# jeongminpark417/COALA-GNN

Measured on AMD Instinct MI355X. Metric: feature-gather GB/s (payload = rows x dim x 4 B delivered per second), IGB-medium GraphSAGE minibatch fetch, higher is better.
Workload: dtype f32

## Files before the change

coala-gnn_amd/csrc/coala_cache.hip:

```cpp
#include <hip/hip_runtime.h>
#include <hip/hip_ext.h>

#include <algorithm>
#include <cstdarg>
#include <cstdio>
#include <cstdlib>
#include <cstring>
#include <new>
#include <type_traits>
#include <utility>
#include <vector>

#include "../../include/coala_hip.h"
#include "coala_internal.h"

namespace {

constexpr uint64_t kEmptyKey = 0xFFFFFFFFFFFFFFFFull;
constexpr uint32_t kLinkMiss = 0x80000000u;
constexpr uint32_t kLinkBad = 0x7FFFFFFFu;
constexpr int kStatBlocks = 2048;
constexpr int kFillSlots = 8;

struct CacheDev {
    void* keys;
    uint64_t* set_cnt;
    uint32_t* color_meta;
    int32_t* color_counters;
    const int32_t* node_color;
    float* lines;
    const float* cold;
    uint64_t num_sets;
    uint64_t num_rows;
    uint32_t cache_dim;
    uint32_t dim;
    uint32_t n_gpus;
    int32_t gshift;
    int32_t sshift;
    uint32_t distributed;
    uint32_t cold_partitioned;
    uint32_t tag32;
    uint64_t* set_head;
    uint32_t* miss_link;
    unsigned long long* stats;
};

__device__ __forceinline__ uint64_t set_of(const CacheDev& c, uint64_t id) {
    uint64_t k = id;
    if (c.distributed) {
        if (c.gshift >= 0) k = id >> c.gshift;
        else if ((id >> 32) == 0) k = (uint32_t)id / c.n_gpus;
        else k = id / c.n_gpus;
    }
    if (c.sshift >= 0) return k & (c.num_sets - 1);
    if ((k >> 32) == 0 && (c.num_sets >> 32) == 0) return (uint32_t)k % (uint32_t)c.num_sets;
    return k % c.num_sets;
}

__device__ __forceinline__ uint64_t cold_row_of(const CacheDev& c, uint64_t id) {
    if (!c.cold_partitioned) return id;
    if (c.gshift >= 0) return id >> c.gshift;
    return id / c.n_gpus;
}

constexpr int kMaxRanges = 64;
struct RangeSet {
    uint32_t n;
    uint32_t total;
    uint32_t begin[kMaxRanges];
    uint32_t vstart[kMaxRanges + 1];
};
__device__ __forceinline__ uint32_t pos_of(const RangeSet& rs, uint32_t v) {
    if (rs.n == 1) return v < rs.total ? rs.begin[0] + v : 0xFFFFFFFFu;
    uint32_t pos = 0xFFFFFFFFu;
    for (uint32_t k = 0; k < rs.n; ++k) {
        const uint32_t a = rs.vstart[k], b = rs.vstart[k + 1];
        if (v >= a && v < b) pos = rs.begin[k] + (v - a);
    }
// ... 48 lines not shown
    static constexpr int UNITS = CD / VEC;
    static constexpr int LPR = UNITS >= 64 ? 64 : UNITS;
    static constexpr int RPP = 64 / LPR;
    static constexpr int VPL = UNITS / LPR;
    static constexpr int PASSES = (VPL >= 16) ? 1 : NP;
    static constexpr int R = RPP * PASSES;
};

constexpr int kK1MinWaves = 4;
constexpr int kK1Passes = 4;
constexpr int64_t kK1SingleMaxChunks = 1 << 20;
constexpr int kK1Waves = 2;
#ifdef COALA_DEV_KNOBS
constexpr int kK1MaxWaves = 4;
#else
constexpr int kK1MaxWaves = kK1Waves;
#endif

template <typename V> __device__ __forceinline__ V nt_load(const V* p) { return __builtin_nontemporal_load(p); }
template <typename V> __device__ __forceinline__ void nt_store(V v, V* p) { __builtin_nontemporal_store(v, p); }

template <int CD, int VEC, typename TAG, int NP, bool FULL, bool REDIR, bool SINGLE>
__global__ __launch_bounds__(64 * kK1MaxWaves, kK1MinWaves) void probe_gather_kernel(const int64_t* __restrict__ idx, float* __restrict__ out,
                                                                    int64_t n, uint32_t gen, uint32_t n_blocks, CacheDev c, Redirect rd) {
    using G = Geo<CD, VEC, NP>;
    using V = typename VecT<VEC>::type;
    using TG = TagGeo<TAG>;
    using TV = typename TG::vec;
    constexpr int R = G::R;
    static_assert(R <= 32, "per-chunk row masks are 32 bits wide");
    if (blockIdx.x == 0 && threadIdx.x < kFillSlots) reinterpret_cast<uint32_t*>(c.stats + 2 * kStatBlocks)[(gen & 1u) * kFillSlots + threadIdx.x] = 0u;
    uint32_t* fill_flag = reinterpret_cast<uint32_t*>(c.stats + 2 * kStatBlocks) + 2 * kFillSlots;
    if (blockIdx.x == 0 && threadIdx.x == kFillSlots) fill_flag[(gen + 1u) & 1u] = 0u;
    constexpr int TSTEPS = (R + TG::SPL - 1) / TG::SPL;
    int lane = threadIdx.x & 63;
#ifdef COALA_DEV_KNOBS
    const int wpb = (int)(blockDim.x >> 6);
#else
    constexpr int wpb = kK1Waves;
#endif
    const int64_t wave = (int64_t)blockIdx.x * wpb + (threadIdx.x >> 6);
    const int64_t n_waves = (int64_t)n_blocks * wpb;
    const int64_t n_chunks = (n + R - 1) / R;
    const uint32_t nunits = c.dim / VEC;
    const TAG* __restrict__ keys = reinterpret_cast<const TAG*>(c.keys);

    struct Ids { uint64_t id[TSTEPS]; bool valid[TSTEPS]; int32_t drow[REDIR ? TSTEPS : 1]; };
    struct Tags { uint64_t id[TSTEPS]; uint32_t set[TSTEPS]; TV kk[TSTEPS]; bool ok[TSTEPS]; bool valid[TSTEPS]; int32_t drow[REDIR ? TSTEPS : 1]; };
    auto load_ids = [&](int64_t chunk) {
        Ids r;
#pragma unroll
        for (int t = 0; t < TSTEPS; ++t) {
            const int q_l = t * TG::SPL + lane / TG::LPS;
            const int64_t i_l = chunk * R + q_l;
            r.valid[t] = (chunk < n_chunks) && (q_l < R) && (i_l < n);
            r.id[t] = r.valid[t] ? (uint64_t)idx[i_l] : 0;
            if (REDIR) {
                int32_t d = -1;
                if (r.valid[t] && i_l >= rd.begin && i_l < rd.end) d = (int32_t)(rd.row_map ? rd.row_map[i_l - rd.begin] : i_l - rd.begin);
                r.drow[t] = d;
            }
        }
        return r;
    };
    auto load_tags = [&](const Ids& ids) {
        Tags r;
// ... 26 lines not shown
        const uint32_t lane_way0 = (uint32_t)((lane % TG::LPS) * TG::KPL);
#pragma unroll
        for (int t = 0; t < TSTEPS; ++t) {
            const TAG want = (TAG)tags.id[t];
            uint32_t way = 0xFFu;
#pragma unroll
            for (int k = TG::KPL - 1; k >= 0; --k)
                if (tags.kk[t][k] == want) way = lane_way0 + (uint32_t)k;
            if (!tags.ok[t]) way = 0xFFu;
            way = umin_u32(way, dpp_u32<0xB1>(way));
            way = umin_u32(way, dpp_u32<0x4E>(way));
            way = umin_u32(way, dpp_u32<0x141>(way));
            if (TG::LPS == 16) way = umin_u32(way, dpp_u32<0x140>(way));
            const bool hit = way != 0xFFu;
            slot_v[t] = tags.set[t] * COALA_WAYS + (way & (COALA_WAYS - 1));
            if (REDIR) drow_v[t] = tags.drow[t];
            hit_b[t] = __ballot(hit);
            bad_l[t] = tags.valid[t] && !tags.ok[t];
            bad_b[t] = __ballot(bad_l[t]);
            lead_l[t] = tags.valid[t] && (lane % TG::LPS) == 0;
            imiss_l[t] = lead_l[t] && tags.ok[t] && !hit;
            prev[t] = 0;
            if (imiss_l[t]) {
                const unsigned long long tag = ((unsigned long long)gen << 32) | (unsigned long long)(base + t * TG::SPL + lane / TG::LPS + 1);
                prev[t] = atomicExch(reinterpret_cast<unsigned long long*>(c.set_head + tags.set[t]), tag);
            }
        }
        {
            bool any = false;
#pragma unroll
            for (int t = 0; t < TSTEPS; ++t) any = any || imiss_l[t] || bad_l[t];
            if (__ballot(any) != 0 && lane == 0) fill_flag[gen & 1u] = 1u;
        }
        auto row_slot = [&](int q) { return (uint32_t)__builtin_amdgcn_readlane((int)slot_v[q / TG::SPL], TG::LPS * (q % TG::SPL)); };
        auto row_hit = [&](int q) { return ((hit_b[q / TG::SPL] >> (TG::LPS * (q % TG::SPL))) & 1) != 0; };
        auto row_bad = [&](int q) { return ((bad_b[q / TG::SPL] >> (TG::LPS * (q % TG::SPL))) & 1) != 0; };
        Ids ids_next2;
        if (!SINGLE) ids_next2 = load_ids(chunk + 2 * n_waves);

        const int sub = (G::RPP == 2) ? (lane >> 5) : 0;
        const int l_in = lane & (G::LPR - 1);
        V val[G::PASSES][G::VPL];
#pragma unroll
        for (int p = 0; p < G::PASSES; ++p) {
            const uint32_t s_a = row_slot(p * G::RPP), s_b = row_slot(p * G::RPP + (G::RPP - 1));
            const bool h_a = row_hit(p * G::RPP), h_b = row_hit(p * G::RPP + (G::RPP - 1));
            const uint32_t s = (G::RPP == 2 && sub) ? s_b : s_a;
            const bool h = (G::RPP == 2 && sub) ? h_b : h_a;
            const V* src = reinterpret_cast<const V*>(c.lines + (uint64_t)s * CD);
#pragma unroll
            for (int v = 0; v < G::VPL; ++v) {
                const uint32_t u = v * G::LPR + l_in;
                if (h && (FULL || u < nunits)) val[p][v] = nt_load(src + u);
            }
        }
        if (!SINGLE) {
            tags = load_tags(ids_next);
            ids_next = ids_next2;
        }
#pragma unroll
        for (int p = 0; p < G::PASSES; ++p) {
            const int q = p * G::RPP + sub;
            const bool h_a = row_hit(p * G::RPP), h_b = row_hit(p * G::RPP + (G::RPP - 1));
            const bool bad_a = row_bad(p * G::RPP), bad_b2 = row_bad(p * G::RPP + (G::RPP - 1));
            const bool h = (G::RPP == 2 && sub) ? h_b : h_a;
            const bool bad = (G::RPP == 2 && sub) ? bad_b2 : bad_a;
            V* dst = reinterpret_cast<V*>(out + (base + q) * (int64_t)c.dim);
            if (REDIR) {
                auto row_drow = [&](int r) { return (int32_t)__builtin_amdgcn_readlane(drow_v[r / TG::SPL], TG::LPS * (r % TG::SPL)); };
                const int32_t dr_a = row_drow(p * G::RPP), dr_b = row_drow(p * G::RPP + (G::RPP - 1));
                const int32_t dr = (G::RPP == 2 && sub) ? dr_b : dr_a;
                if (dr >= 0) dst = reinterpret_cast<V*>(rd.out + (int64_t)dr * (int64_t)c.dim);
            }
#pragma unroll
            for (int v = 0; v < G::VPL; ++v) {
                const uint32_t u = v * G::LPR + l_in;
                if (FULL || u < nunits) {
                    if (h) dst[u] = val[p][v];
                    else if (bad) dst[u] = V(0.0f);
                }
            }
        }
#pragma unroll
        for (int t = 0; t < TSTEPS; ++t) {
            if (lead_l[t]) {
                uint32_t w = 0u;
                if (imiss_l[t]) w = kLinkMiss | (((uint32_t)(prev[t] >> 32) == gen) ? (uint32_t)prev[t] : 0u);
                else if (bad_l[t]) w = kLinkBad;
                c.miss_link[base + t * TG::SPL + lane / TG::LPS] = w;
            }
        }
        if (SINGLE) break;
    }
}

enum { kOpAssign = 0, kOpAdd = 1, kOpAdagrad = 2 };
constexpr int kStatWriteBad = 2 * kStatBlocks + kFillSlots + 1;
constexpr int kStatWords = kStatWriteBad + 1;

template <int OP> __device__ __forceinline__ float write_op(float x, float old, float& st, float a, float eps) {
    if (OP == kOpAssign) return x;
    if (OP == kOpAdd) return __builtin_fmaf(a, x, old);
    const float s = st + x * x;
    st = s;
    return old - a * x / (__builtin_sqrtf(s) + eps);
}
template <int OP> __device__ __forceinline__ vfloat4 write_op(vfloat4 x, vfloat4 old, vfloat4& st, float a, float eps) {
    vfloat4 r;
#pragma unroll
    for (int k = 0; k < 4; ++k) {
        float s = st[k];
        r[k] = write_op<OP>(x[k], old[k], s, a, eps);
        st[k] = s;
    }
    return r;
}

template <int CD, int VEC, typename TAG, int OP>
__global__ __launch_bounds__(256) void write_rows_kernel(const int64_t* __restrict__ ids, const float* __restrict__ src, float* __restrict__ state,
                                                         int64_t n, float a, float eps, CacheDev c) {
    using G = Geo<CD, VEC, 1>;
    using V = typename VecT<VEC>::type;
    using TG = TagGeo<TAG>;
    using TV = typename TG::vec;
    constexpr int R = TG::SPL;
    static_assert(R % G::RPP == 0, "a chunk is a whole number of passes");
    const int lane = threadIdx.x & 63;
    const int64_t wave = (int64_t)blockIdx.x * (blockDim.x >> 6) + (threadIdx.x >> 6);
    const int64_t n_waves = (int64_t)gridDim.x * (blockDim.x >> 6);
    const int64_t n_chunks = (n + R - 1) / R;
    const uint32_t nunits = c.dim / VEC;
// ... 33 lines not shown
            if (!live) continue;
            const int64_t i = chunk * R + q;
            const V* xs = reinterpret_cast<const V*>(src + i * (int64_t)c.dim);
            V* cold_row = reinterpret_cast<V*>(cold + id * (uint64_t)c.dim);
            V* st_row = OP == kOpAdagrad ? reinterpret_cast<V*>(state + id * (uint64_t)c.dim) : nullptr;
            float* set_lines = c.lines + (uint64_t)set * COALA_WAYS * CD;
            const V* old_row = m ? reinterpret_cast<const V*>(set_lines + (uint64_t)__builtin_ctz(m) * CD) : cold_row;
            V x[G::VPL], old[G::VPL], st[G::VPL];
#pragma unroll
            for (int v = 0; v < G::VPL; ++v) {
                const uint32_t u = v * G::LPR + l_in;
                x[v] = V(0.0f); old[v] = V(0.0f); st[v] = V(0.0f);
                if (u < nunits) {
                    x[v] = nt_load(xs + u);
                    if (OP != kOpAssign) old[v] = old_row[u];
                    if (OP == kOpAdagrad) st[v] = st_row[u];
                }
            }
#pragma unroll
            for (int v = 0; v < G::VPL; ++v) {
                const uint32_t u = v * G::LPR + l_in;
                if (u < nunits) {
                    const V nv = write_op<OP>(x[v], old[v], st[v], a, eps);
                    if (OP == kOpAdagrad) st_row[u] = st[v];
                    cold_row[u] = nv;
                    for (uint32_t mm = m; mm; mm &= mm - 1)
                        reinterpret_cast<V*>(set_lines + (uint64_t)__builtin_ctz(mm) * CD)[u] = nv;
                }
            }
        }
    }
}


template <int CD, int VEC, bool REDIR = false, int NP = 4>
__global__ __launch_bounds__(256) void miss_fill_kernel(CacheDev c, const int64_t* __restrict__ idx, float* __restrict__ out,
                                                        int tile_rows, int sparse_max, uint32_t gen, RangeSet rs, Redirect rd, int dyn_slot) {
    using G = Geo<CD, VEC, NP>;
    using V = typename VecT<VEC>::type;
    constexpr int R = G::R;
    const int lane = threadIdx.x & 63;
    const int64_t wave = (int64_t)blockIdx.x * (blockDim.x >> 6) + (threadIdx.x >> 6);
    const int64_t n_waves = (int64_t)gridDim.x * (blockDim.x >> 6);
    const int64_t n_tiles = ((int64_t)rs.total + tile_rows - 1) / tile_rows;
    const int chunks_per_tile = tile_rows / R;
    const uint32_t nunits = c.dim / VEC;
    const int sub = (G::RPP == 2) ? (lane >> 5) : 0;
    const int l_in = lane & (G::LPR - 1);
    uint32_t my_miss = 0, my_bad = 0;

    constexpr int U = 8;
    uint32_t* ticket = reinterpret_cast<uint32_t*>(c.stats + 2 * kStatBlocks) + (dyn_slot < 0 ? 0 : dyn_slot);
    const bool dyn = dyn_slot >= 0;
    if (reinterpret_cast<const uint32_t*>(c.stats + 2 * kStatBlocks)[2 * kFillSlots + (gen & 1u)] == 0u) return;
    const int64_t n_deal = dyn ? 1 : n_waves;
    const int64_t even8 = n_tiles / (n_waves * 8);
    const int claim_min = even8 < 1 ? 1 : (even8 > U ? U : (int)even8);
    int claim = claim_min;
    for (int64_t unit = dyn ? -1 : wave;;) {
      int64_t claim_end = n_tiles;
      if (dyn) {
          uint32_t t = 0;
          if (lane == 0) t = atomicAdd(ticket, (uint32_t)claim);
          unit = (int64_t)(uint32_t)__builtin_amdgcn_readfirstlane((int)t);
          if (unit >= n_tiles) break;
          claim_end = unit + claim < n_tiles ? unit + claim : n_tiles;
          claim = claim * 2 > 4 * U ? 4 * U : claim * 2;
      } else if (unit >= n_tiles) break;
     for (int64_t tile0 = unit; tile0 < claim_end; tile0 += n_deal * U) {
      const int n_here = dyn ? (int)(claim_end - tile0 < U ? claim_end - tile0 : U) : U;
      uint64_t st_pack = 0;
#pragma unroll
      for (int u = 0; u < U; ++u) {
          const int64_t tile = tile0 + u * n_deal;
          const uint32_t p = (u < n_here && tile < n_tiles && lane < tile_rows) ? pos_of(rs, (uint32_t)(tile * tile_rows + lane)) : 0xFFFFFFFFu;
          const uint32_t w = (p != 0xFFFFFFFFu) ? c.miss_link[p] : 0u;
          const uint64_t v = (w == 0u) ? 0u : ((w & kLinkMiss) ? 1u : 2u);
          st_pack |= v << (8 * u);
      }
      if (!__ballot(st_pack != 0)) continue;
      uint32_t slot_l = 0, win_l = 0;
      uint64_t id_l = 0;
      int64_t drow_l = 0;
      auto rank_at = [&](uint32_t pos) {
          id_l = (uint64_t)idx[pos];
          drow_l = (int64_t)pos;
          if (REDIR && (int64_t)pos >= rd.begin && (int64_t)pos < rd.end)
              drow_l = -((rd.row_map ? rd.row_map[(int64_t)pos - rd.begin] : (int64_t)pos - rd.begin) + 1);
          const uint64_t set = set_of(c, id_l);
          uint32_t cur = (uint32_t)c.set_head[set];
          uint32_t total = 0, rank = 0;
          while (cur) {
              const uint32_t p2 = cur - 1;
              ++total;
              rank += (p2 < pos) ? 1u : 0u;
              cur = c.miss_link[p2] & ~kLinkMiss;
          }
          const uint64_t cv = __hip_atomic_load(c.set_cnt + set, __ATOMIC_RELAXED, __HIP_MEMORY_SCOPE_AGENT);
          const uint32_t cnt0 = ((uint32_t)(cv >> 32) == gen) ? (uint32_t)cv - total : (uint32_t)cv;
          if (rank == 0) __hip_atomic_store(c.set_cnt + set, ((uint64_t)gen << 32) | (uint32_t)(cnt0 + total), __ATOMIC_RELAXED, __HIP_MEMORY_SCOPE_AGENT);
          const uint32_t way = (cnt0 + rank) & (COALA_WAYS - 1);
          slot_l = (uint32_t)(set * COALA_WAYS) + way;
          win_l = (rank + COALA_WAYS >= total) ? 1u : 0u;
          if (win_l) {
              if (c.tag32) reinterpret_cast<uint32_t*>(c.keys)[slot_l] = (uint32_t)id_l;
              else reinterpret_cast<uint64_t*>(c.keys)[slot_l] = id_l;
              if (c.color_counters) {
                  const int32_t col = c.node_color[id_l];
                  atomicSub(c.color_counters + c.color_meta[slot_l], 1);
                  atomicAdd(c.color_counters + col, 1);
                  c.color_meta[slot_l] = (uint32_t)col;
              }
          }
      };
      auto move_group = [&](const int (&srcl)[G::PASSES], const bool (&live)[G::PASSES]) {
          V val[G::PASSES][G::VPL];
          uint32_t slot_[G::PASSES];
          uint64_t id[G::PASSES];
          int64_t drow[G::PASSES];
          bool winner[G::PASSES];
#pragma unroll
          for (int p = 0; p < G::PASSES; ++p) {
              slot_[p] = (uint32_t)__shfl((int)slot_l, srcl[p]);
              winner[p] = __shfl((int)win_l, srcl[p]) != 0;
              id[p] = shfl64(id_l, srcl[p]);
              drow[p] = (int64_t)shfl64((uint64_t)drow_l, srcl[p]);
          }
#pragma unroll
          for (int p = 0; p < G::PASSES; ++p) {
              const V* src = reinterpret_cast<const V*>(c.cold + cold_row_of(c, id[p]) * (uint64_t)c.dim);
#pragma unroll
              for (int v = 0; v < G::VPL; ++v) {
                  const uint32_t u = v * G::LPR + l_in;
                  if (live[p] && u < nunits) val[p][v] = nt_load(src + u);
              }
          }
#pragma unroll
          for (int p = 0; p < G::PASSES; ++p) {
              V* dst = (REDIR && drow[p] < 0) ? reinterpret_cast<V*>(rd.out + (uint64_t)(-(drow[p] + 1)) * c.dim)
                                              : reinterpret_cast<V*>(out + (uint64_t)drow[p] * c.dim);
              V* line = reinterpret_cast<V*>(c.lines + (uint64_t)slot_[p] * CD);
#pragma unroll
              for (int v = 0; v < G::VPL; ++v) {
                  const uint32_t u = v * G::LPR + l_in;
                  if (live[p] && u < nunits) {
                      nt_store(val[p][v], dst + u);
                      if (winner[p]) nt_store(val[p][v], line + u);
                  }
              }
          }
      };
      auto stream_holders = [&](uint64_t holders) {
          int srcl[G::PASSES];
          bool live[G::PASSES];
          while (holders) {
#pragma unroll
              for (int p = 0; p < G::PASSES; ++p) {
                  int l0 = -1, l1 = -1;
                  if (holders) { l0 = __builtin_ctzll(holders); holders &= holders - 1; }
                  if (G::RPP == 2 && holders) { l1 = __builtin_ctzll(holders); holders &= holders - 1; }
                  const int l = (G::RPP == 2 && sub) ? l1 : l0;
                  live[p] = l >= 0;
                  srcl[p] = l >= 0 ? l : 0;
              }
              move_group(srcl, live);
          }
      };
      uint64_t mmask[U];
      uint32_t total_miss = 0, worst = 0;
#pragma unroll
      for (int u = 0; u < U; ++u) {
          const uint8_t st = (uint8_t)(st_pack >> (8 * u));
          mmask[u] = __ballot(st == 1);
          my_miss += (st == 1);
          my_bad += (st == 2);
          const uint32_t cnt = (uint32_t)__builtin_popcountll(mmask[u]);
          total_miss += cnt;
          worst = cnt > worst ? cnt : worst;
      }
      if (!total_miss) continue;
      claim = claim_min;
      if (total_miss <= 64 && (int)worst <= sparse_max) {
          uint32_t k = (uint32_t)lane;
// ... 15 lines not shown
          stream_holders(total_miss >= 64 ? ~0ull : ((1ull << total_miss) - 1ull));
          continue;
      }
#pragma nounroll
      for (int u = 0; u < U; ++u) {
        const uint8_t st = (uint8_t)(st_pack >> (8 * u));
        const uint64_t tile_mask = __ballot(st == 1);
        if (!tile_mask) continue;
        const uint32_t pos_l = st ? pos_of(rs, (uint32_t)((tile0 + u * n_deal) * tile_rows + lane)) : 0u;
        if (__builtin_popcountll(tile_mask) <= sparse_max) {
            if (st == 1) rank_at(pos_l);
            stream_holders(tile_mask);
        } else {
            int srcl[G::PASSES];
            bool live[G::PASSES];
            for (int ck = 0; ck < chunks_per_tile; ++ck) {
                const uint32_t live_mask = (uint32_t)(tile_mask >> (ck * R)) & ((1u << R) - 1u);
                if (!live_mask) continue;
                const int lane0 = ck * R;
                if (st == 1 && lane >= lane0 && lane < lane0 + R) rank_at(pos_l);
#pragma unroll
                for (int p = 0; p < G::PASSES; ++p) {
                    const int q = p * G::RPP + sub;
                    live[p] = (live_mask >> q) & 1;
                    srcl[p] = lane0 + q;
                }
                move_group(srcl, live);
            }
        }
      }
     }
      if (!dyn) break;
    }
    __shared__ uint32_t s_m[256 / 64], s_b[256 / 64];
    for (int off = 32; off > 0; off >>= 1) { my_miss += __shfl_down(my_miss, off); my_bad += __shfl_down(my_bad, off); }
    if (lane == 0) { s_m[threadIdx.x >> 6] = my_miss; s_b[threadIdx.x >> 6] = my_bad; }
    __syncthreads();
    if (threadIdx.x == 0) {
        uint32_t m = 0, b = 0;
        for (int w = 0; w < (int)(blockDim.x >> 6); ++w) { m += s_m[w]; b += s_b[w]; }
        if (m) c.stats[2 * blockIdx.x] += m;
        if (b) c.stats[2 * blockIdx.x + 1] += b;
    }
}

template <int CD, int VEC, int NP = 4>
__global__ __launch_bounds__(256) void scatter_rows_kernel(float* __restrict__ out, const float* __restrict__ src,
                                                           const int64_t* __restrict__ map, RangeSet rs, uint32_t dim) {
    using G = Geo<CD, VEC, NP>;
    using V = typename VecT<VEC>::type;
    constexpr int R = G::R;
    const int lane = threadIdx.x & 63;
    const int64_t wave = (int64_t)blockIdx.x * (blockDim.x >> 6) + (threadIdx.x >> 6);
    const int64_t n_waves = (int64_t)gridDim.x * (blockDim.x >> 6);
    const int64_t n_chunks = ((int64_t)rs.total + R - 1) / R;
    const uint32_t nunits = dim / VEC;
    const int sub = (G::RPP == 2) ? (lane >> 5) : 0;
    const int l_in = lane & (G::LPR - 1);
    for (int64_t chunk = wave; chunk < n_chunks; chunk += n_waves) {
        const int64_t base = chunk * R;
        V val[G::PASSES][G::VPL];
        int64_t d[G::PASSES];
#pragma unroll
        for (int p = 0; p < G::PASSES; ++p) {
            const int64_t vr = base + p * G::RPP + sub;
            const uint32_t r = (vr < (int64_t)rs.total) ? pos_of(rs, (uint32_t)vr) : 0xFFFFFFFFu;
            d[p] = (r != 0xFFFFFFFFu) ? map[r] : -1;
            const V* s = reinterpret_cast<const V*>(src + (int64_t)r * (int64_t)dim);
#pragma unroll
            for (int v = 0; v < G::VPL; ++v) {
                const uint32_t u = v * G::LPR + l_in;
                if (d[p] >= 0 && u < nunits) val[p][v] = nt_load(s + u);
            }
        }
#pragma unroll
        for (int p = 0; p < G::PASSES; ++p) {
// ... 182 lines not shown
};

namespace {

#define fail coala_fail_
#define HIPCHK COALA_HIPCHK

int follow_stream(coala_cache* h, hipStream_t s) {
    if (h->order_set && h->order_stream != s) {
        if (!h->order_ev) HIPCHK(hipEventCreateWithFlags(&h->order_ev, hipEventDisableTiming));
        if (hipEventRecord(h->order_ev, h->order_stream) == hipSuccess) HIPCHK(hipStreamWaitEvent(s, h->order_ev, 0));
        else (void)hipGetLastError();
    }
    h->order_stream = s;
    h->order_set = true;
    return COALA_OK;
}

int ilog2_exact(uint64_t v) {
    if (v == 0 || (v & (v - 1))) return -1;
    int s = 0;
    while ((1ull << s) != v) ++s;
    return s;
}

int ensure_scratch(coala_cache* h, uint64_t n, hipStream_t s) {
    if (n <= h->cap) return COALA_OK;
    HIPCHK(hipStreamSynchronize(s));
    uint64_t cap = h->cap ? h->cap : 1024;
    while (cap < n) cap *= 2;
    if (h->d.miss_link) HIPCHK(hipFree(h->d.miss_link));
    h->d.miss_link = nullptr;
    HIPCHK(hipMalloc((void**)&h->d.miss_link, cap * sizeof(uint32_t)));
    h->cap = cap;
    return COALA_OK;
}

hipEvent_t take_event(coala_cache* h) {
    if (!h->ev_pool.empty()) {
        hipEvent_t e = h->ev_pool.back();
        h->ev_pool.pop_back();
        return e;
    }
    hipEvent_t e = nullptr;
    if (hipEventCreate(&e) != hipSuccess) return nullptr;
    return e;
}

void drain_events(coala_cache* h) {
    for (auto& p : h->ev_live) {
        float ms = 0.f;
        if (hipEventSynchronize(p.b) == hipSuccess && hipEventElapsedTime(&ms, p.a, p.b) == hipSuccess) {
            if (p.kind == 0) { h->prof.gather_ms += ms; h->prof.gather_launches++; h->prof.gather_rows += p.rows; }
            else { h->prof.fill_ms += ms; h->prof.fill_launches++; }
        }
        h->ev_pool.push_back(p.a);
        h->ev_pool.push_back(p.b);
    }
    h->ev_live.clear();
}

struct ProfScope {
    coala_cache* h; hipStream_t s; int kind; uint64_t rows; hipEvent_t a = nullptr, b = nullptr; bool on;
    hipEvent_t xa = nullptr, xb = nullptr;
    ProfScope(coala_cache* h_, hipStream_t s_, int kind_, uint64_t rows_, hipEvent_t xa_ = nullptr, hipEvent_t xb_ = nullptr)
        : h(h_), s(s_), kind(kind_), rows(rows_), xa(xa_), xb(xb_) {
// ... 151 lines not shown
        }
        h->gen = 0;
        {
            hipPointerAttribute_t attr;
            const bool host_tier = hipPointerGetAttributes(&attr, cfg->cold_table) == hipSuccess && attr.type == hipMemoryTypeHost;
            (void)hipGetLastError();
            h->host_tier = host_tier;
            h->shape = launch_shape(d.cache_dim, host_tier);
#ifdef COALA_DEV_KNOBS
            apply_dev_knobs(h->shape);
#endif
        }
        if (cfg->max_batch) rc = ensure_scratch(h, cfg->max_batch, nullptr);
    } while (0);
    if (rc == COALA_OK && hipDeviceSynchronize() != hipSuccess) rc = fail(COALA_EHIP, "device sync failed after create");
    if (rc != COALA_OK) {
        coala_cache_destroy(h);
        return rc;
    }
    *out = h;
    return COALA_OK;
}

int coala_cache_destroy(coala_cache_t* h) {
    if (!h) return COALA_OK;
    (void)hipSetDevice(h->cfg.device);
    (void)hipDeviceSynchronize();
    drain_events(h);
    for (auto e : h->ev_pool) (void)hipEventDestroy(e);
    for (auto e : h->fev)
        if (e) (void)hipEventDestroy(e);
    CacheDev& d = h->d;
    void* ptrs[] = {d.keys, d.set_cnt, d.color_meta, d.set_head, d.stats, d.lines, d.color_counters,
                    h->node_color_dev, d.miss_link,
                    h->wave_counts, h->route_bases};
    for (void* p : ptrs)
        if (p) (void)hipFree(p);
    if (h->color_pin) (void)hipHostFree(h->color_pin);
    if (h->color_pin_async) (void)hipHostFree(h->color_pin_async);
    if (h->color_ev) (void)hipEventDestroy(h->color_ev);
    if (h->order_ev) (void)hipEventDestroy(h->order_ev);
    delete h;
    return COALA_OK;
}

int64_t coala_cache_row_dim(const coala_cache_t* h) { return h ? (int64_t)h->d.dim : 0; }

int coala_cache_fetch_events(coala_cache_t* h, int enable) {
    if (!h) return fail(COALA_EINVAL, "null handle");
    h->fetch_events = enable != 0;
    if (!h->fetch_events) h->last_begin = h->last_end = nullptr;
    return COALA_OK;
}

int coala_cache_last_fetch_events(const coala_cache_t* h, void** begin_ev, void** end_ev) {
    if (!h) return fail(COALA_EINVAL, "null handle");
    if (begin_ev) *begin_ev = (void*)h->last_begin;
    if (end_ev) *end_ev = (void*)h->last_end;
    return COALA_OK;
}

int coala_stream_wait_event(void* stream, void* event) {
    if (!event) return fail(COALA_EINVAL, "null event");
    HIPCHK(hipStreamWaitEvent((hipStream_t)stream, (hipEvent_t)event, 0));
    return COALA_OK;
}

// ... 56 lines not shown
    const int64_t whole_b = 0, whole_e = n;
    if (phases == kPhaseBoth) { begins = &whole_b; ends = &whole_e; n_ranges = 1; }
    int64_t fill_rows = 0;
    if (phases & kPhaseFill) {
        if (n_ranges < 0 || (n_ranges > 0 && (!begins || !ends))) return fail(COALA_EINVAL, "bad fill ranges");
        std::vector<std::pair<int64_t, int64_t>> add;
        for (int k = 0; k < n_ranges; ++k) {
            if (begins[k] < 0 || begins[k] > ends[k] || ends[k] > n)
                return fail(COALA_EINVAL, "fill range [%lld, %lld) outside the batch of %lld rows", (long long)begins[k], (long long)ends[k], (long long)n);
            if (ends[k] > begins[k]) add.emplace_back(begins[k], ends[k]);
        }
        if (phases == kPhaseFill) {
            std::vector<std::pair<int64_t, int64_t>> all = h->open_filled;
            all.insert(all.end(), add.begin(), add.end());
            std::sort(all.begin(), all.end());
            for (size_t k = 1; k < all.size(); ++k)
                if (all[k].first < all[k - 1].second)
                    return fail(COALA_EINVAL, "fill range [%lld, %lld) overlaps positions that were already filled in this batch", (long long)all[k].first, (long long)all[k].second);
            h->open_filled.swap(all);
        }
        for (auto& r : add) fill_rows += r.second - r.first;
        if (fill_rows == 0 && !(phases & kPhaseProbe)) return COALA_OK;
    }
    hipStream_t s = (hipStream_t)stream;
    HIPCHK(hipSetDevice(h->cfg.device));
    if (int rc_ = follow_stream(h, s)) return rc_;
    int rc = ensure_scratch(h, (uint64_t)n, s);
    if (rc) return rc;
    if (phases & kPhaseProbe) {
        h->fill_launches = 0;
        if (++h->gen == 0) {
            HIPCHK(hipMemsetAsync(h->d.set_head, 0, h->d.num_sets * 8, s));
            HIPCHK(hipMemset2DAsync(reinterpret_cast<char*>(h->d.set_cnt) + 4, 8, 0, 4, h->d.num_sets, s));
            h->gen = 1;
        }
        if (!(phases & kPhaseFill)) {
            h->open_batch_rows = n;
            h->open_filled.clear();
            h->open_filled_rows = 0;
            h->open_redirect = rd;
        }
    }
    const uint32_t gen = h->gen;
    const bool redir = rd.end > rd.begin;
    const bool vec4 = (h->d.dim % 4 == 0) && aligned16(out) && aligned16(h->d.cold) && (!redir || aligned16(rd.out));
    CacheDev d = h->d;
    if (force_dist) d.distributed = 1u;
    hipEvent_t fe_begin = nullptr, fe_end = nullptr;
    if (h->fetch_events && phases == kPhaseBoth && !(h->cfg.flags & COALA_FLAG_PROFILE)) {
        if (h->fev.empty()) h->fev.assign(2 * (size_t)coala_cache::kFetchRing, nullptr);
        const size_t slot = (size_t)(h->fev_calls % coala_cache::kFetchRing);
        for (size_t k = 2 * slot; k < 2 * slot + 2; ++k)
            if (!h->fev[k]) HIPCHK(hipEventCreate(&h->fev[k]));
        fe_begin = h->fev[2 * slot];
        fe_end = h->fev[2 * slot + 1];
    }
    const bool own_ring = fe_begin != nullptr;
    if (!own_ring && !(h->cfg.flags & COALA_FLAG_PROFILE)) {
        fe_begin = (phases & kPhaseProbe) ? ext_begin : nullptr;
        fe_end = (phases & kPhaseFill) ? ext_end : nullptr;
    }
    int n_sets = 0, set_no = 0;
    if ((phases & kPhaseFill) && fill_rows > 0) {
        int live = 0;
        for (int k = 0; k < n_ranges; ++k) live += ends[k] > begins[k];
        n_sets = (live + kMaxRanges - 1) / kMaxRanges;
    }
    rc = dispatch_geo(d.cache_dim, vec4, [&](auto geo) -> int {
        constexpr int CD = geo_cd(geo);
        constexpr int VEC = geo_vec(geo);
        using G = Geo<CD, VEC>;
        if (phases & kPhaseProbe) {
            ProfScope ps(h, s, 0, (uint64_t)n, fe_begin, nullptr);
            if (rode) rode[0] = ps.on ? ps.a : fe_begin;
            const bool full = (VEC == 4) && ((int)d.dim == CD);
            auto launch_k1 = [&](auto tag_c, auto np_c) {
                using TAG = decltype(tag_c);
                constexpr int NP = decltype(np_c)::value;
                constexpr int NPR = (Geo<CD, VEC, NP>::R > 8) ? NP / 2 : NP;
                using GK = Geo<CD, VEC, NP>;
                using GR = Geo<CD, VEC, NPR>;
                const int64_t chunks = redir ? (n + GR::R - 1) / GR::R : (n + GK::R - 1) / GK::R;
                const LaunchShape& ls = h->shape;
                const bool single = ls.k1_single && chunks <= kK1SingleMaxChunks;
                const dim3 grid(grid_for(chunks, ls.k1_waves, single ? (int)((kK1SingleMaxChunks + ls.k1_waves - 1) / ls.k1_waves) : ls.k1_grid_cap)), block(64 * ls.k1_waves);
                auto pick = [&](auto single_c) {
                    constexpr bool S = decltype(single_c)::value;
                    if (redir) return full ? probe_gather_kernel<CD, VEC, TAG, NPR, true, true, S> : probe_gather_kernel<CD, VEC, TAG, NPR, false, true, S>;
                    return full ? probe_gather_kernel<CD, VEC, TAG, NP, true, false, S> : probe_gather_kernel<CD, VEC, TAG, NP, false, false, S>;
                };
                ps.launch(single ? pick(std::true_type{}) : pick(std::false_type{}), grid, block, idx, out, n, gen, (uint32_t)grid.x, d, rd);
            };
#ifdef COALA_DEV_KNOBS
            if (h->shape.k1_passes) {
                auto by_np = [&](auto tag_c) {
                    switch (h->shape.k1_passes) {
                        case 2: launch_k1(tag_c, std::integral_constant<int, 2>{}); break;
                        case 8: launch_k1(tag_c, std::integral_constant<int, 8>{}); break;
                        case 16: launch_k1(tag_c, std::integral_constant<int, (Geo<CD, VEC, 16>::R <= 32 ? 16 : 8)>{}); break;
                        default: launch_k1(tag_c, std::integral_constant<int, 4>{}); break;
                    }
                };
                if (d.tag32) by_np(uint32_t{}); else by_np(uint64_t{});
            } else
#endif
            if (d.tag32) launch_k1(uint32_t{}, std::integral_constant<int, kK1Passes>{});
            else launch_k1(uint64_t{}, std::integral_constant<int, kK1Passes>{});
        }
        if ((phases & kPhaseFill) && fill_rows > 0) {
            const int tile_rows = h->shape.k2_tile_rows > 0 ? h->shape.k2_tile_rows : G::R;
            return for_each_range_set(begins, ends, n_ranges, [&](const RangeSet& rs) -> int {
                const bool last_set = ++set_no == n_sets;
                ProfScope ps(h, s, 2, 0, nullptr, last_set ? fe_end : nullptr);
                if (rode && last_set) rode[1] = ps.on ? ps.b : fe_end;
                const int64_t tiles = ((int64_t)rs.total + tile_rows - 1) / tile_rows;
                const dim3 grid(grid_for(tiles, 4, h->shape.k2_grid_cap));
                const int64_t waves = (int64_t)grid.x * 4;
                int dyn_slot = -1;
                if (h->shape.k2_unit_tiles > 0 && tiles > waves && tiles < 0x7FFFFFFF && h->fill_launches < kFillSlots)
                    dyn_slot = (int)((gen & 1u) * kFillSlots) + h->fill_launches;
                h->fill_launches++;
                if (redir) ps.launch(miss_fill_kernel<CD, VEC, true>, grid, dim3(256), d, idx, out, tile_rows, h->shape.k2_sparse_max, gen, rs, rd, dyn_slot);
                else ps.launch(miss_fill_kernel<CD, VEC, false>, grid, dim3(256), d, idx, out, tile_rows, h->shape.k2_sparse_max, gen, rs, rd, dyn_slot);
                return COALA_OK;
            });
        }
        return COALA_OK;
    });
    if (rc) return rc;
    if (own_ring) {
        h->last_begin = fe_begin;
        h->last_end = fe_end;
        h->fev_calls++;
    }
    if (phases & kPhaseProbe) h->rows_total += (uint64_t)n;
    if (phases == kPhaseFill) {
        h->open_filled_rows += fill_rows;
        if (h->open_filled_rows == h->open_batch_rows) {
            h->open_batch_rows = -1;
            h->open_filled.clear();
            h->open_filled_rows = 0;
        }
// ... 190 lines not shown
}

int coala_cache_color_counts_async(coala_cache_t* h, int32_t n_entries, void* stream) {
    if (!h) return fail(COALA_EINVAL, "null argument");
    if (n_entries < 0 || n_entries > h->cfg.num_colors + 1) return fail(COALA_EINVAL, "n_entries=%d exceeds num_colors+1=%d", n_entries, h->cfg.num_colors + 1);
    if (h->color_pending >= 0) return fail(COALA_EINVAL, "a colour-counter snapshot is already pending: call coala_cache_color_counts_finish first");
    HIPCHK(hipSetDevice(h->cfg.device));
    if (int rc_ = follow_stream(h, (hipStream_t)stream)) return rc_;
    if (h->d.color_counters) {
        if (!h->color_pin_async) HIPCHK(hipHostMalloc((void**)&h->color_pin_async, ((size_t)h->cfg.num_colors + 1) * 4, hipHostMallocDefault));
        if (!h->color_ev) HIPCHK(hipEventCreateWithFlags(&h->color_ev, hipEventDisableTiming));
        HIPCHK(hipMemcpyAsync(h->color_pin_async, h->d.color_counters, (size_t)n_entries * 4, hipMemcpyDeviceToHost, (hipStream_t)stream));
        HIPCHK(hipEventRecord(h->color_ev, (hipStream_t)stream));
    }
    h->color_pending = n_entries;
    return COALA_OK;
}

int coala_cache_color_counts_finish(coala_cache_t* h, int32_t* dst, int32_t n_entries) {
    if (!h || !dst) return fail(COALA_EINVAL, "null argument");
    if (h->color_pending < 0 || n_entries != h->color_pending) return fail(COALA_EINVAL, "no pending snapshot of %d entries", n_entries);
    if (!h->d.color_counters) {
        memset(dst, 0, (size_t)n_entries * 4);
    } else {
        HIPCHK(hipSetDevice(h->cfg.device));
        HIPCHK(hipEventSynchronize(h->color_ev));
        memcpy(dst, h->color_pin_async, (size_t)n_entries * 4);
    }
    h->color_pending = -1;
    return COALA_OK;
}

static int read_stats(coala_cache_t* h, hipStream_t s, uint64_t* hit, uint64_t* miss, uint64_t* bad, bool reset) {
    std::vector<unsigned long long> part((size_t)kStatWords);
    HIPCHK(hipMemcpyAsync(part.data(), h->d.stats, part.size() * 8, hipMemcpyDeviceToHost, s));
    if (reset) {
        HIPCHK(hipMemsetAsync(h->d.stats, 0, (size_t)kStatBlocks * 2 * 8, s));
        HIPCHK(hipMemsetAsync(h->d.stats + kStatWriteBad, 0, 8, s));
    }
    HIPCHK(hipStreamSynchronize(s));
    uint64_t m = 0, b = 0;
    for (int i = 0; i < kStatBlocks; ++i) { m += part[2 * i]; b += part[2 * i + 1]; }
    *miss = m;
    *bad = b + part[kStatWriteBad];
    *hit = h->rows_total - m - b;
    if (reset) { h->cum_hit += *hit; h->cum_miss += m; h->rows_total = 0; }
    return COALA_OK;
}

int coala_cache_stats(coala_cache_t* h, uint64_t* hit, uint64_t* miss, uint64_t* range_errors, int reset, void* stream) {
    if (!h) return fail(COALA_EINVAL, "null handle");
    HIPCHK(hipSetDevice(h->cfg.device));
    if (int rc_ = follow_stream(h, (hipStream_t)stream)) return rc_;
    uint64_t v0, v1, v2;
    int rc = read_stats(h, (hipStream_t)stream, &v0, &v1, &v2, reset != 0);
    if (rc) return rc;
    if (hit) *hit = v0;
    if (miss) *miss = v1;
    if (range_errors) *range_errors = v2;
    return COALA_OK;
}

int coala_cache_dump(coala_cache_t* h, uint64_t* keys, uint32_t* set_cnt, uint32_t* color_meta, void* stream) {
    if (!h) return fail(COALA_EINVAL, "null handle");
    hipStream_t s = (hipStream_t)stream;
    HIPCHK(hipSetDevice(h->cfg.device));
    if (int rc_ = follow_stream(h, (hipStream_t)stream)) return rc_;
    const uint64_t slots = h->d.num_sets * COALA_WAYS;
    HIPCHK(hipStreamSynchronize(s));
    if (keys) {
        if (h->d.tag32) {
            uint32_t* narrow = reinterpret_cast<uint32_t*>(keys);
            HIPCHK(hipMemcpy(narrow, h->d.keys, slots * 4, hipMemcpyDeviceToHost));
            for (uint64_t k = slots; k-- > 0;) keys[k] = narrow[k] == 0xFFFFFFFFu ? kEmptyKey : (uint64_t)narrow[k];
        } else {
// ... 42 lines not shown
```

Before: 81.65.

## Compact miss positions into sharded lists and fill only listed misses

The probe kernel now appends each wave's miss positions into one of 64 sharded compact lists, using per-shard atomic counters, and counts bad rows directly. When both phases run with a host tier, a new list-driven fill kernel prefix-sums the shard counters and processes only the listed misses with ticket-based dynamic scheduling. It no longer scans range sets for misses. This removes fill-kernel work proportional to all rows in favour of work proportional to misses, at the cost of extra atomics and list writes in the probe kernel and a new device buffer.

After: 82.66, median of 6. +1.2%, better.

```diff
diff --git a/coala-gnn_amd/csrc/coala_cache.hip b/coala-gnn_amd/csrc/coala_cache.hip
--- a/coala-gnn_amd/csrc/coala_cache.hip
+++ b/coala-gnn_amd/csrc/coala_cache.hip
@@ -43,7 +43,20 @@
     uint64_t* set_head;
     uint32_t* miss_link;
     unsigned long long* stats;
+    uint32_t* miss_list;
+    uint32_t list_sub;
 };
+
+constexpr int kListShards = 64;
+constexpr int kListStride = 64;
+constexpr int kStatWriteBad = 2 * kStatBlocks + kFillSlots + 1;
+constexpr int kStatProbeBad = kStatWriteBad + 1;
+constexpr int kStatHostWords = kStatProbeBad + 1;
+constexpr int kStatList = (kStatHostWords + 31) & ~31;
+constexpr int kStatWords = kStatList + 2 * kListShards * kListStride / 2;
+__device__ __forceinline__ uint32_t* list_counter(const CacheDev& c, uint32_t parity, uint32_t shard) {
+    return reinterpret_cast<uint32_t*>(c.stats + kStatList) + (parity * kListShards + shard) * kListStride;
+}
 
 __device__ __forceinline__ uint64_t set_of(const CacheDev& c, uint64_t id) {
     uint64_t k = id;
@@ -158,6 +171,7 @@
     if (blockIdx.x == 0 && threadIdx.x < kFillSlots) reinterpret_cast<uint32_t*>(c.stats + 2 * kStatBlocks)[(gen & 1u) * kFillSlots + threadIdx.x] = 0u;
     uint32_t* fill_flag = reinterpret_cast<uint32_t*>(c.stats + 2 * kStatBlocks) + 2 * kFillSlots;
     if (blockIdx.x == 0 && threadIdx.x == kFillSlots) fill_flag[(gen + 1u) & 1u] = 0u;
+    if (blockIdx.x == 0 && threadIdx.x < kListShards) *list_counter(c, (gen + 1u) & 1u, threadIdx.x) = 0u;
     constexpr int TSTEPS = (R + TG::SPL - 1) / TG::SPL;
     int lane = threadIdx.x & 63;
 #ifdef COALA_DEV_KNOBS
@@ -250,6 +264,18 @@
             for (int t = 0; t < TSTEPS; ++t) any = any || imiss_l[t] || bad_l[t];
             if (__ballot(any) != 0 && lane == 0) fill_flag[gen & 1u] = 1u;
         }
+        const uint32_t shard = (uint32_t)chunk & (kListShards - 1);
+        uint32_t list_at = 0;
+        if (c.list_sub) {
+            uint32_t n_miss = 0, n_bad = 0;
+#pragma unroll
+            for (int t = 0; t < TSTEPS; ++t) {
+                n_miss += (uint32_t)__builtin_popcountll(__ballot(imiss_l[t]));
+                n_bad += (uint32_t)__builtin_popcountll(__ballot(bad_l[t] && lead_l[t]));
+            }
+            if (n_miss && lane == 0) list_at = atomicAdd(list_counter(c, gen & 1u, shard), n_miss);
+            if (n_bad && lane == 0) atomicAdd(c.stats + kStatProbeBad, (unsigned long long)n_bad);
+        }
         auto row_slot = [&](int q) { return (uint32_t)__builtin_amdgcn_readlane((int)slot_v[q / TG::SPL], TG::LPS * (q % TG::SPL)); };
         auto row_hit = [&](int q) { return ((hit_b[q / TG::SPL] >> (TG::LPS * (q % TG::SPL))) & 1) != 0; };
         auto row_bad = [&](int q) { return ((bad_b[q / TG::SPL] >> (TG::LPS * (q % TG::SPL))) & 1) != 0; };
@@ -308,13 +334,20 @@
                 c.miss_link[base + t * TG::SPL + lane / TG::LPS] = w;
             }
         }
+        if (c.list_sub) {
+            uint32_t at = (uint32_t)__builtin_amdgcn_readfirstlane((int)list_at);
+#pragma unroll
+            for (int t = 0; t < TSTEPS; ++t) {
+                const uint64_t mb = __ballot(imiss_l[t]);
+                if (imiss_l[t]) c.miss_list[shard * c.list_sub + at + (uint32_t)__builtin_popcountll(mb & ((1ull << lane) - 1ull))] = (uint32_t)(base + t * TG::SPL + lane / TG::LPS);
+                at += (uint32_t)__builtin_popcountll(mb);
+            }
+        }
         if (SINGLE) break;
     }
 }
 
 enum { kOpAssign = 0, kOpAdd = 1, kOpAdagrad = 2 };
-constexpr int kStatWriteBad = 2 * kStatBlocks + kFillSlots + 1;
-constexpr int kStatWords = kStatWriteBad + 1;
 
 template <int OP> __device__ __forceinline__ float write_op(float x, float old, float& st, float a, float eps) {
     if (OP == kOpAssign) return x;
@@ -414,6 +447,77 @@
     }
 }
 
+
+
+__device__ __forceinline__ void rank_row(const CacheDev& c, uint32_t gen, uint32_t pos, uint64_t id, uint32_t& slot, uint32_t& win) {
+    const uint64_t set = set_of(c, id);
+    uint32_t cur = (uint32_t)c.set_head[set];
+    uint32_t total = 0, rank = 0;
+    while (cur) {
+        const uint32_t p2 = cur - 1;
+        ++total;
+        rank += (p2 < pos) ? 1u : 0u;
+        cur = c.miss_link[p2] & ~kLinkMiss;
+    }
+    const uint64_t cv = __hip_atomic_load(c.set_cnt + set, __ATOMIC_RELAXED, __HIP_MEMORY_SCOPE_AGENT);
+    const uint32_t cnt0 = ((uint32_t)(cv >> 32) == gen) ? (uint32_t)cv - total : (uint32_t)cv;
+    if (rank == 0) __hip_atomic_store(c.set_cnt + set, ((uint64_t)gen << 32) | (uint32_t)(cnt0 + total), __ATOMIC_RELAXED, __HIP_MEMORY_SCOPE_AGENT);
+    const uint32_t way = (cnt0 + rank) & (COALA_WAYS - 1);
+    slot = (uint32_t)(set * COALA_WAYS) + way;
+    win = (rank + COALA_WAYS >= total) ? 1u : 0u;
+    if (win) {
+        if (c.tag32) reinterpret_cast<uint32_t*>(c.keys)[slot] = (uint32_t)id;
+        else reinterpret_cast<uint64_t*>(c.keys)[slot] = id;
+        if (c.color_counters) {
+            const int32_t col = c.node_color[id];
+            atomicSub(c.color_counters + c.color_meta[slot], 1);
+            atomicAdd(c.color_counters + col, 1);
+            c.color_meta[slot] = (uint32_t)col;
+        }
+    }
+}
+template <typename G, typename V>
+__device__ __forceinline__ void cold_load(const CacheDev& c, const uint64_t (&id)[G::PASSES], const bool (&live)[G::PASSES], int l_in, uint32_t nunits,
+                                          V (&val)[G::PASSES][G::VPL]) {
+#pragma unroll
+    for (int p = 0; p < G::PASSES; ++p) {
+        const V* src = reinterpret_cast<const V*>(c.cold + cold_row_of(c, id[p]) * (uint64_t)c.dim);
+#pragma unroll
+        for (int v = 0; v < G::VPL; ++v) {
+            const uint32_t u = v * G::LPR + l_in;
+            if (live[p] && u < nunits) val[p][v] = nt_load(src + u);
+        }
+    }
+}
+template <int CD, typename G, typename V>
+__device__ __forceinline__ void fill_store(const CacheDev& c, V* const (&dst)[G::PASSES], const uint32_t (&slot)[G::PASSES], const bool (&winner)[G::PASSES],
+                                           const bool (&live)[G::PASSES], int l_in, uint32_t nunits, const V (&val)[G::PASSES][G::VPL]) {
+#pragma unroll
+    for (int p = 0; p < G::PASSES; ++p) {
+        V* line = reinterpret_cast<V*>(c.lines + (uint64_t)slot[p] * CD);
+#pragma unroll
+        for (int v = 0; v < G::VPL; ++v) {
+            const uint32_t u = v * G::LPR + l_in;
+            if (live[p] && u < nunits) {
+                nt_store(val[p][v], dst[p] + u);
+                if (winner[p]) nt_store(val[p][v], line + u);
+            }
+        }
+    }
+}
+__device__ __forceinline__ void add_block_stats(const CacheDev& c, uint32_t my_miss, uint32_t my_bad) {
+    __shared__ uint32_t s_m[256 / 64], s_b[256 / 64];
+    const int lane = threadIdx.x & 63;
+    for (int off = 32; off > 0; off >>= 1) { my_miss += __shfl_down(my_miss, off); my_bad += __shfl_down(my_bad, off); }
+    if (lane == 0) { s_m[threadIdx.x >> 6] = my_miss; s_b[threadIdx.x >> 6] = my_bad; }
+    __syncthreads();
+    if (threadIdx.x == 0) {
+        uint32_t m = 0, b = 0;
+        for (int w = 0; w < (int)(blockDim.x >> 6); ++w) { m += s_m[w]; b += s_b[w]; }
+        if (m) c.stats[2 * blockIdx.x] += m;
+        if (b) c.stats[2 * blockIdx.x + 1] += b;
+    }
+}
 
 template <int CD, int VEC, bool REDIR = false, int NP = 4>
 __global__ __launch_bounds__(256) void miss_fill_kernel(CacheDev c, const int64_t* __restrict__ idx, float* __restrict__ out,
@@ -469,31 +573,7 @@
           drow_l = (int64_t)pos;
           if (REDIR && (int64_t)pos >= rd.begin && (int64_t)pos < rd.end)
               drow_l = -((rd.row_map ? rd.row_map[(int64_t)pos - rd.begin] : (int64_t)pos - rd.begin) + 1);
-          const uint64_t set = set_of(c, id_l);
-          uint32_t cur = (uint32_t)c.set_head[set];
-          uint32_t total = 0, rank = 0;
-          while (cur) {
-              const uint32_t p2 = cur - 1;
-              ++total;
-              rank += (p2 < pos) ? 1u : 0u;
-              cur = c.miss_link[p2] & ~kLinkMiss;
-          }
-          const uint64_t cv = __hip_atomic_load(c.set_cnt + set, __ATOMIC_RELAXED, __HIP_MEMORY_SCOPE_AGENT);
-          const uint32_t cnt0 = ((uint32_t)(cv >> 32) == gen) ? (uint32_t)cv - total : (uint32_t)cv;
-          if (rank == 0) __hip_atomic_store(c.set_cnt + set, ((uint64_t)gen << 32) | (uint32_t)(cnt0 + total), __ATOMIC_RELAXED, __HIP_MEMORY_SCOPE_AGENT);
-          const uint32_t way = (cnt0 + rank) & (COALA_WAYS - 1);
-          slot_l = (uint32_t)(set * COALA_WAYS) + way;
-          win_l = (rank + COALA_WAYS >= total) ? 1u : 0u;
-          if (win_l) {
-              if (c.tag32) reinterpret_cast<uint32_t*>(c.keys)[slot_l] = (uint32_t)id_l;
-              else reinterpret_cast<uint64_t*>(c.keys)[slot_l] = id_l;
-              if (c.color_counters) {
-                  const int32_t col = c.node_color[id_l];
-                  atomicSub(c.color_counters + c.color_meta[slot_l], 1);
-                  atomicAdd(c.color_counters + col, 1);
-                  c.color_meta[slot_l] = (uint32_t)col;
-              }
-          }
+          rank_row(c, gen, pos, id_l, slot_l, win_l);
       };
       auto move_group = [&](const int (&srcl)[G::PASSES], const bool (&live)[G::PASSES]) {
           V val[G::PASSES][G::VPL];
@@ -501,6 +581,7 @@
           uint64_t id[G::PASSES];
           int64_t drow[G::PASSES];
           bool winner[G::PASSES];
+          V* dst[G::PASSES];
 #pragma unroll
           for (int p = 0; p < G::PASSES; ++p) {
               slot_[p] = (uint32_t)__shfl((int)slot_l, srcl[p]);
@@ -508,29 +589,12 @@
               id[p] = shfl64(id_l, srcl[p]);
               drow[p] = (int64_t)shfl64((uint64_t)drow_l, srcl[p]);
           }
-#pragma unroll
-          for (int p = 0; p < G::PASSES; ++p) {
-              const V* src = reinterpret_cast<const V*>(c.cold + cold_row_of(c, id[p]) * (uint64_t)c.dim);
-#pragma unroll
-              for (int v = 0; v < G::VPL; ++v) {
-                  const uint32_t u = v * G::LPR + l_in;
-                  if (live[p] && u < nunits) val[p][v] = nt_load(src + u);
-              }
-          }
-#pragma unroll
-          for (int p = 0; p < G::PASSES; ++p) {
-              V* dst = (REDIR && drow[p] < 0) ? reinterpret_cast<V*>(rd.out + (uint64_t)(-(drow[p] + 1)) * c.dim)
+          cold_load<G>(c, id, live, l_in, nunits, val);
+#pragma unroll
+          for (int p = 0; p < G::PASSES; ++p)
+              dst[p] = (REDIR && drow[p] < 0) ? reinterpret_cast<V*>(rd.out + (uint64_t)(-(drow[p] + 1)) * c.dim)
                                               : reinterpret_cast<V*>(out + (uint64_t)drow[p] * c.dim);
-              V* line = reinterpret_cast<V*>(c.lines + (uint64_t)slot_[p] * CD);
-#pragma unroll
-              for (int v = 0; v < G::VPL; ++v) {
-                  const uint32_t u = v * G::LPR + l_in;
-                  if (live[p] && u < nunits) {
-                      nt_store(val[p][v], dst + u);
-                      if (winner[p]) nt_store(val[p][v], line + u);
-                  }
-              }
-          }
+          fill_store<CD, G>(c, dst, slot_, winner, live, l_in, nunits, val);
       };
       auto stream_holders = [&](uint64_t holders) {
           int srcl[G::PASSES];
@@ -612,16 +676,75 @@
      }
       if (!dyn) break;
     }
-    __shared__ uint32_t s_m[256 / 64], s_b[256 / 64];
-    for (int off = 32; off > 0; off >>= 1) { my_miss += __shfl_down(my_miss, off); my_bad += __shfl_down(my_bad, off); }
-    if (lane == 0) { s_m[threadIdx.x >> 6] = my_miss; s_b[threadIdx.x >> 6] = my_bad; }
-    __syncthreads();
-    if (threadIdx.x == 0) {
-        uint32_t m = 0, b = 0;
-        for (int w = 0; w < (int)(blockDim.x >> 6); ++w) { m += s_m[w]; b += s_b[w]; }
-        if (m) c.stats[2 * blockIdx.x] += m;
-        if (b) c.stats[2 * blockIdx.x + 1] += b;
-    }
+    add_block_stats(c, my_miss, my_bad);
+}
+
+template <int CD, int VEC, int NP = 4>
+__global__ __launch_bounds__(256) void miss_fill_list_kernel(CacheDev c, const int64_t* __restrict__ idx, float* __restrict__ out, uint32_t gen) {
+    using G = Geo<CD, VEC, NP>;
+    using V = typename VecT<VEC>::type;
+    constexpr int R = G::R;
+    const int lane = threadIdx.x & 63;
+    const uint32_t wave = blockIdx.x * (blockDim.x >> 6) + (threadIdx.x >> 6);
+    const uint32_t n_waves = gridDim.x * (blockDim.x >> 6);
+    const uint32_t nunits = c.dim / VEC;
+    const int sub = (G::RPP == 2) ? (lane >> 5) : 0;
+    const int l_in = lane & (G::LPR - 1);
+    static_assert(kListShards == 64, "one list counter per lane");
+    const uint32_t cnt_l = __hip_atomic_load(list_counter(c, gen & 1u, (uint32_t)lane), __ATOMIC_RELAXED, __HIP_MEMORY_SCOPE_AGENT);
+    uint32_t incl = cnt_l;
+    for (int off = 1; off < 64; off <<= 1) {
+        const uint32_t v = __shfl_up(incl, off);
+        if (lane >= off) incl += v;
+    }
+    const uint32_t excl = incl - cnt_l;
+    const uint32_t total = (uint32_t)__builtin_amdgcn_readlane((int)incl, 63);
+    if (total == 0) return;
+    const uint32_t n_groups = (total + R - 1) / R;
+    uint32_t* ticket = reinterpret_cast<uint32_t*>(c.stats + 2 * kStatBlocks) + (gen & 1u) * kFillSlots;
+    uint32_t my_miss = 0;
+    for (uint32_t g = wave; g < n_groups;) {
+        uint32_t pos_l = 0;
+#pragma unroll
+        for (int j = 0; j < R; ++j) {
+            const uint32_t e = g * R + j;
+            const uint32_t s = (uint32_t)__builtin_popcountll(__ballot(incl <= e)) & 63u;
+            const uint32_t off = e - (uint32_t)__builtin_amdgcn_readlane((int)excl, (int)s);
+            if (lane == j && e < total) pos_l = c.miss_list[s * c.list_sub + off];
+        }
+        const bool have = lane < R && g * R + (uint32_t)lane < total;
+        const uint64_t id_l = have ? (uint64_t)idx[pos_l] : 0;
+        uint64_t id[G::PASSES];
+        uint32_t pos[G::PASSES];
+        bool live[G::PASSES];
+        V val[G::PASSES][G::VPL];
+#pragma unroll
+        for (int p = 0; p < G::PASSES; ++p) {
+            const int q = p * G::RPP + sub;
+            live[p] = g * R + (uint32_t)q < total;
+            id[p] = shfl64(id_l, q);
+            pos[p] = (uint32_t)__shfl((int)pos_l, q);
+        }
+        cold_load<G>(c, id, live, l_in, nunits, val);
+        uint32_t t = 0;
+        if (lane == 0) t = atomicAdd(ticket, 1u);
+        uint32_t slot_l = 0, win_l = 0;
+        if (have) rank_row(c, gen, pos_l, id_l, slot_l, win_l);
+        uint32_t slot[G::PASSES];
+        bool winner[G::PASSES];
+        V* dst[G::PASSES];
+#pragma unroll
+        for (int p = 0; p < G::PASSES; ++p) {
+            const int q = p * G::RPP + sub;
+            slot[p] = (uint32_t)__shfl((int)slot_l, q);
+            winner[p] = __shfl((int)win_l, q) != 0;
+            dst[p] = reinterpret_cast<V*>(out + (uint64_t)pos[p] * c.dim);
+        }
+        fill_store<CD, G>(c, dst, slot, winner, live, l_in, nunits, val);
+        if (lane == 0) my_miss += (total - g * R < (uint32_t)R) ? total - g * R : (uint32_t)R;
+        g = n_waves + (uint32_t)__builtin_amdgcn_readfirstlane((int)t);
+    }
+    add_block_stats(c, my_miss, 0u);
 }
 
 template <int CD, int VEC, int NP = 4>
@@ -870,6 +993,10 @@
     if (h->d.miss_link) HIPCHK(hipFree(h->d.miss_link));
     h->d.miss_link = nullptr;
     HIPCHK(hipMalloc((void**)&h->d.miss_link, cap * sizeof(uint32_t)));
+    if (h->d.miss_list) HIPCHK(hipFree(h->d.miss_list));
+    h->d.miss_list = nullptr;
+    h->d.list_sub = (uint32_t)(cap / kListShards) + 32u;
+    HIPCHK(hipMalloc((void**)&h->d.miss_list, (uint64_t)kListShards * h->d.list_sub * sizeof(uint32_t)));
     h->cap = cap;
     return COALA_OK;
 }
@@ -1087,7 +1214,7 @@
         if (e) (void)hipEventDestroy(e);
     CacheDev& d = h->d;
     void* ptrs[] = {d.keys, d.set_cnt, d.color_meta, d.set_head, d.stats, d.lines, d.color_counters,
-                    h->node_color_dev, d.miss_link,
+                    h->node_color_dev, d.miss_link, d.miss_list,
                     h->wave_counts, h->route_bases};
     for (void* p : ptrs)
         if (p) (void)hipFree(p);
@@ -1210,6 +1337,7 @@
         if (++h->gen == 0) {
             HIPCHK(hipMemsetAsync(h->d.set_head, 0, h->d.num_sets * 8, s));
             HIPCHK(hipMemset2DAsync(reinterpret_cast<char*>(h->d.set_cnt) + 4, 8, 0, 4, h->d.num_sets, s));
+            HIPCHK(hipMemsetAsync(h->d.stats + kStatList, 0, (size_t)(kStatWords - kStatList) * 8, s));
             h->gen = 1;
         }
         if (!(phases & kPhaseFill)) {
@@ -1224,6 +1352,8 @@
     const bool vec4 = (h->d.dim % 4 == 0) && aligned16(out) && aligned16(h->d.cold) && (!redir || aligned16(rd.out));
     CacheDev d = h->d;
     if (force_dist) d.distributed = 1u;
+    const bool list_form = phases == kPhaseBoth && h->host_tier;
+    if (!list_form) d.list_sub = 0;
     hipEvent_t fe_begin = nullptr, fe_end = nullptr;
     if (h->fetch_events && phases == kPhaseBoth && !(h->cfg.flags & COALA_FLAG_PROFILE)) {
         if (h->fev.empty()) h->fev.assign(2 * (size_t)coala_cache::kFetchRing, nullptr);
@@ -1286,6 +1416,13 @@
             else launch_k1(uint64_t{}, std::integral_constant<int, kK1Passes>{});
         }
         if ((phases & kPhaseFill) && fill_rows > 0) {
+            if (list_form) {
+                ProfScope ps(h, s, 2, 0, nullptr, fe_end);
+                if (rode) rode[1] = ps.on ? ps.b : fe_end;
+                h->fill_launches++;
+                ps.launch(miss_fill_list_kernel<CD, VEC>, dim3(grid_for((n + G::R - 1) / G::R, 4, h->shape.k2_grid_cap)), dim3(256), d, idx, out, gen);
+                return COALA_OK;
+            }
             const int tile_rows = h->shape.k2_tile_rows > 0 ? h->shape.k2_tile_rows : G::R;
             return for_each_range_set(begins, ends, n_ranges, [&](const RangeSet& rs) -> int {
                 const bool last_set = ++set_no == n_sets;
@@ -1542,15 +1679,16 @@
 }
 
 static int read_stats(coala_cache_t* h, hipStream_t s, uint64_t* hit, uint64_t* miss, uint64_t* bad, bool reset) {
-    std::vector<unsigned long long> part((size_t)kStatWords);
+    std::vector<unsigned long long> part((size_t)kStatHostWords);
     HIPCHK(hipMemcpyAsync(part.data(), h->d.stats, part.size() * 8, hipMemcpyDeviceToHost, s));
     if (reset) {
         HIPCHK(hipMemsetAsync(h->d.stats, 0, (size_t)kStatBlocks * 2 * 8, s));
-        HIPCHK(hipMemsetAsync(h->d.stats + kStatWriteBad, 0, 8, s));
+        HIPCHK(hipMemsetAsync(h->d.stats + kStatWriteBad, 0, 2 * 8, s));
     }
     HIPCHK(hipStreamSynchronize(s));
     uint64_t m = 0, b = 0;
     for (int i = 0; i < kStatBlocks; ++i) { m += part[2 * i]; b += part[2 * i + 1]; }
+    b += part[kStatProbeBad];
     *miss = m;
     *bad = b + part[kStatWriteBad];
     *hit = h->rows_total - m - b;
```
